# jjjkkyz/NU-NeRF

Hardware: AMD Instinct MI355X
Metric: train rays/sec (higher is better)
Workload: dtype f32

## Files before the change

nu_nerf_amd/csrc/gemm_tn.hip:

```cpp
#include "gemm_epi.h"

__device__ unsigned long long nu_dbg_clk[2];

#define NU_TN_BATCH_MAX 16
struct NuGemmTNBatch {
    NuGemmTN p[NU_TN_BATCH_MAX];
    int blk0[NU_TN_BATCH_MAX + 1];
    int n, pad_;
};
static __device__ __forceinline__ int tn_batch_decode(const NuGemmTNBatch& b, int tile_edge, int& bx, int& split) {
    int pi = 0;
    for (int i = 1; i < b.n; ++i) pi = ((int)blockIdx.x >= b.blk0[i]) ? i : pi;
    const int tiles = ((b.p[pi].N1 + tile_edge - 1) / tile_edge) * ((b.p[pi].N2 + tile_edge - 1) / tile_edge);
    const int local = (int)blockIdx.x - b.blk0[pi];
    split = local / tiles;
    bx = local - split * tiles;
    return pi;
}

template <bool BIG, int PREC>
static __device__ __forceinline__ void tn_body(const NuGemmTN& g, const int bx, const int split, const int grp) {
    constexpr bool BF16 = PREC == 1;
    constexpr bool SPLIT = PREC == 2;
    constexpr int kPlane = 128 * NT_LDSH;
    __shared__ __attribute__((aligned(16))) float smem[SPLIT ? 1 : 2][SPLIT ? 3 * kPlane : 128 * NT_LDS];
    __bf16* const hA = reinterpret_cast<__bf16*>(&smem[0][0]);
    __bf16* const hB = hA + (SPLIT ? 3 : 1) * kPlane;

    const int tid = threadIdx.x;
    const int lane = tid & 63;
    const int wid = tid >> 6;
    const int wr = wid >> 1, wc = wid & 1;
    const int t2 = (g.N2 + 127) / 128;
    const int n1t = bx / t2, n2t = bx - n1t * t2;
    const int n1_0 = n1t * 128, n2_0 = n2t * 128;
    const int N1p = ((g.N1 + 127) / 128) * 128, N2p = t2 * 128;

    int rows_per = (g.P + g.S - 1) / g.S;
    rows_per = ((rows_per + TBK - 1) / TBK) * TBK;
    const int p_begin = split * rows_per;
    int p_end = p_begin + rows_per;
    p_end = p_end < g.P ? p_end : g.P;
    const int ntile = p_end > p_begin ? (p_end - p_begin + TBK - 1) / TBK : 0;
    const int npair = g.A1 ? 2 : 1;
    const int total = ntile * npair;

    const int c = tid & 127;
    const int kg = tid >> 7;
    const bool do_bias = (g.bias_slab != nullptr) && (n2t == 0);

    f32x16 acc[2][2];
#pragma unroll
    for (int i = 0; i < 2; ++i)
#pragma unroll
        for (int j = 0; j < 2; ++j)
#pragma unroll
            for (int r = 0; r < 16; ++r) acc[i][j][r] = 0.0f;

    f32x4 ra4[4], rb4[4];
    int nvalid = 16;
    bool pend_pair0 = true;
    float bs = 0.f;
    auto load_tile = [&](int t) {
        const int pair = t >= ntile ? 1 : 0;
        const int kt = t - pair * ntile;
        const bool a16 = BF16 && (g.bf16 & (pair ? NU_TN_A1_16 : NU_TN_A0_16)) != 0;
        const bool b16 = BF16 && (g.bf16 & (pair ? NU_TN_B1_16 : NU_TN_B0_16)) != 0;
        const unsigned eA = a16 ? 2u : 4u, eB = b16 ? 2u : 4u;
        const char* __restrict__ A = (const char*)(pair ? g.A1 : g.A0) + (long long)grp * (pair ? g.sA1 : g.sA0) * eA;
        const char* __restrict__ B = (const char*)(pair ? g.B1 : g.B0) + (long long)grp * (pair ? g.sB1 : g.sB0) * eB;
        const int lda = pair ? g.lda1 : g.lda0;
        const int ldb = pair ? g.ldb1 : g.ldb0;
        int ca = n1_0 + c, cb = n2_0 + c;
        ca = ca < lda ? ca : lda - 1;
        cb = cb < ldb ? cb : ldb - 1;
        const int pbase = p_begin + kt * TBK + kg * 16;
        nvalid = p_end - pbase;
        pend_pair0 = pair == 0;
#pragma unroll
        for (int i = 0; i < 4; ++i)
#pragma unroll
            for (int e = 0; e < 4; ++e) {
                int pr = pbase + 4 * i + e;
                pr = pr < p_end ? pr : p_end - 1;
                const char* pa;
                const char* pb;
                if (BIG) {
                    pa = A + ((long long)pr * lda + ca) * eA;
                    pb = B + ((long long)pr * ldb + cb) * eB;
                } else {
                    pa = A + ((unsigned)pr * (unsigned)lda + (unsigned)ca) * eA;
                    pb = B + ((unsigned)pr * (unsigned)ldb + (unsigned)cb) * eB;
                }
                ra4[i][e] = a16 ? __uint_as_float((unsigned)*reinterpret_cast<const unsigned short*>(pa) << 16) : *reinterpret_cast<const float*>(pa);
                rb4[i][e] = b16 ? __uint_as_float((unsigned)*reinterpret_cast<const unsigned short*>(pb) << 16) : *reinterpret_cast<const float*>(pb);
            }
    };
    auto store_tile = [&]() {
#pragma unroll
        for (int i = 0; i < 4; ++i)
#pragma unroll
// ... 655 lines not shown
        TN_SLOT(F1, 2, TN_LD2(1, 2))
        TN_SLOT(F1, 3, TN_READS(F0, cur, 2))
        TN_SLOT(F0, 0, TN_ST(2))
        TN_SLOT(F0, 1, TN_ST(3))
        TN_SLOT(F0, 2, TN_LD2(2, 0))
        TN_SLOT(F0, 3, TN_READS(F1, cur, 3))
        __syncthreads();
        TN_SLOT(F1, 0, TN_LD2(2, 2))
        TN_SLOT(F1, 1, TN_LD2(3, 0))
        TN_SLOT(F1, 2, TN_LD2(3, 2))
        TN_SLOT(F1, 3, TN_READS(F0, cur ^ 1, 0))
        nvalid = nvalid_ld; pend_pair0 = pair0_ld;
        cur ^= 1;
    }
#undef TN_PIN
#undef TN_M
#undef TN_SLOT
#undef TN_SLOT_
#undef TN_RDA
#undef TN_RDB
#undef TN_READS
#undef TN_LD2
#undef TN_ST

    float* __restrict__ slab = g.slab + (long long)grp * g.sSlab + (long long)split * N1p * N2p;
#pragma unroll
    for (int tm = 0; tm < 2; ++tm)
#pragma unroll
        for (int tn = 0; tn < 4; ++tn) {
            const int col = n2_0 + wc * 128 + tn * 32 + li;
#pragma unroll
            for (int r = 0; r < 16; ++r) {
                const int row = n1_0 + wr * 64 + tm * 32 + (r & 3) + 8 * (r >> 2) + 4 * lh;
                slab[(long long)row * N2p + col] = acc[tm][tn][r];
            }
        }
    if (do_bias) {
        float* red = &smem[0][0][0];
        red[kg * T + c] = bs;
        __syncthreads();
        if (tid < T) g.bias_slab[(long long)grp * g.sBiasSlab + (long long)split * N1p + n1_0 + tid] = red[tid] + red[T + tid];
    }
}

template <bool BIG>
__global__ __launch_bounds__(512, 2) void gemm_tn2_kernel(NuGemmTN g) { tn2_body<BIG>(g, blockIdx.x, blockIdx.y, blockIdx.z); }
template <bool BIG>
__global__ __launch_bounds__(512, 2) void gemm_tn2b_kernel(NuGemmTNBatch b) {
    int bx, split;
    const int pi = tn_batch_decode(b, 256, bx, split);
    tn2_body<BIG>(b.p[pi], bx, split, 0);
}

static bool nu_tn_big_tile(int N1, int N2, int groups, int prec, int S) {
    if ((prec & 3) == 2 || (N1 % 256) != 0 || (N2 % 256) != 0) return false;
    return (long long)(N1 / 256) * (N2 / 256) * (groups > 0 ? groups : 1) * S >= 192;
}
extern "C" int nu_wgrad_pick_split(int P, int N1, int N2, int groups, int prec) {
    if (groups < 1) groups = 1;
    const int rows_min = P <= 8192 ? 128 : 256;
    const int cap = (P + rows_min - 1) / rows_min > 0 ? (P + rows_min - 1) / rows_min : 1;
    if ((N1 % 256) == 0 && (N2 % 256) == 0) {
        int S = 256 / ((N1 / 256) * (N2 / 256) * groups);
        if (S < 1) S = 1;
        if (S > cap) S = cap;
        if (nu_tn_big_tile(N1, N2, groups, prec, S)) return S;
    }
    int S = 512 / (nu_cdiv(N1, 128) * nu_cdiv(N2, 128) * groups);
    if (S < 1) S = 1;
    if (S > cap) S = cap;
    return S;
}

int nu_gemm_tn_launch(const NuGemmTN& g, hipStream_t stream) {
    if (g.N1 <= 0 || g.N2 <= 0 || g.S <= 0) return NU_ERR_ARG;
    if ((g.lda0 & 3) || (g.ldb0 & 3) || (g.A1 && ((g.lda1 & 3) || (g.ldb1 & 3)))) return NU_ERR_ARG;
    const int prec = g.bf16 & 3;
    if (prec == 3 || ((g.bf16 & ~3) && prec != 1)) return NU_ERR_ARG;
    const bool big_tile = nu_tn_big_tile(g.N1, g.N2, g.groups, g.bf16, g.S);
    const long long max_ld = (g.lda0 > g.ldb0 ? g.lda0 : g.ldb0) > (g.A1 ? (g.lda1 > g.ldb1 ? g.lda1 : g.ldb1) : 0)
                                 ? (g.lda0 > g.ldb0 ? g.lda0 : g.ldb0) : (g.lda1 > g.ldb1 ? g.lda1 : g.ldb1);
    const bool big = (long long)g.P * max_ld * 4 >= (1LL << 32);
    if (prec == 0 && big_tile) {
        dim3 grid2((g.N1 / 256) * (g.N2 / 256), g.S, g.groups > 0 ? g.groups : 1);
        if (big) hipLaunchKernelGGL((gemm_tn2_kernel<true>), grid2, dim3(512), 0, stream, g);
        else hipLaunchKernelGGL((gemm_tn2_kernel<false>), grid2, dim3(512), 0, stream, g);
        return nu_launch_status();
    }
    dim3 grid(nu_cdiv(g.N1, 128) * nu_cdiv(g.N2, 128), g.S, g.groups > 0 ? g.groups : 1), block(256);
    if (prec == 1) {
        auto ok = [](const float* p, int ld, bool h) { return p == nullptr || ((((uintptr_t)p) & 15) == 0 && ld >= 8 && (!h || (ld & 7) == 0)); };
        const bool vec = ok(g.A0, g.lda0, g.bf16 & NU_TN_A0_16) && ok(g.B0, g.ldb0, g.bf16 & NU_TN_B0_16) &&
                         ok(g.A1, g.lda1, g.bf16 & NU_TN_A1_16) && ok(g.B1, g.ldb1, g.bf16 & NU_TN_B1_16) &&
                         ((g.sA0 | g.sB0 | g.sA1 | g.sB1) & 7) == 0;
        if (vec) {
            if (big_tile) {
                dim3 grid2((g.N1 / 256) * (g.N2 / 256), g.S, g.groups > 0 ? g.groups : 1);
                hipLaunchKernelGGL(gemm_tn16x256_kernel, grid2, dim3(512), 0, stream, g);
            } else {
                hipLaunchKernelGGL(gemm_tn16_kernel, grid, block, 0, stream, g);
            }
            return nu_launch_status();
        }
    }
    if (big) {
        if (prec == 2) hipLaunchKernelGGL((gemm_tn_kernel<true, 2>), grid, block, 0, stream, g);
        else if (prec == 1) hipLaunchKernelGGL((gemm_tn_kernel<true, 1>), grid, block, 0, stream, g);
        else hipLaunchKernelGGL((gemm_tn_kernel<true, 0>), grid, block, 0, stream, g);
    } else {
        if (prec == 2) hipLaunchKernelGGL((gemm_tn_kernel<false, 2>), grid, block, 0, stream, g);
        else if (prec == 1) hipLaunchKernelGGL((gemm_tn_kernel<false, 1>), grid, block, 0, stream, g);
        else hipLaunchKernelGGL((gemm_tn_kernel<false, 0>), grid, block, 0, stream, g);
    }
    return nu_launch_status();
}

struct NuReduceBatch {
    NuReduceDesc d[NU_REDUCE_MAX];
    int n;
};

__global__ __launch_bounds__(256) void slab_reduce_batched_kernel(NuReduceBatch b) {
    __shared__ float red[256];
    int di = 0;
    for (int i = 1; i < b.n; ++i) di = ((int)blockIdx.x >= b.d[i].blk_begin) ? i : di;
    const float* __restrict__ slab = b.d[di].slab;
    float* __restrict__ out = b.d[di].out;
    const int S = b.d[di].S, N1 = b.d[di].N1, N2 = b.d[di].N2, rs = b.d[di].rs, G = b.d[di].G;
    const long long ss = b.d[di].ss;
    const int opb = 256 / G;
    const int o = threadIdx.x % opb, g = threadIdx.x / opb;
    const int idx = ((int)blockIdx.x - b.d[di].blk_begin) * opb + o;
    const bool live = idx < N1 * N2;
    float v = 0.f;
    int n1 = 0, n2 = 0;
    if (live) {
        n1 = idx / N2;
        n2 = idx - n1 * N2;
        const float* p = slab + (long long)n1 * rs + n2;
        float s0 = 0.f, s1 = 0.f, s2 = 0.f, s3 = 0.f;
        int s = g;
        for (; s + 3 * G < S; s += 4 * G) {
            s0 += p[(long long)s * ss];
            s1 += p[(long long)(s + G) * ss];
            s2 += p[(long long)(s + 2 * G) * ss];
            s3 += p[(long long)(s + 3 * G) * ss];
        }
        for (; s < S; s += G) s0 += p[(long long)s * ss];
        v = (s0 + s1) + (s2 + s3);
    }
    if (G > 1) {
        red[threadIdx.x] = v;
        __syncthreads();
        if (g == 0)
            for (int gg = 1; gg < G; ++gg) v += red[gg * opb + o];
    }
    if (live && g == 0) {
        float* q = out + (long long)n1 * b.d[di].ldo + n2;
        v *= b.d[di].alpha;
        *q = b.d[di].accumulate ? *q + v : v;
    }
}

static int nu_reduce_launch_chunk(const NuReduceDesc* descs, int n, hipStream_t stream) {
    NuReduceBatch b;
    int blocks = 0;
    for (int i = 0; i < n; ++i) {
        b.d[i] = descs[i];
        const long long nout = (long long)descs[i].N1 * descs[i].N2;
        int G = 1;
        while (G < 16 && nout * G < 16384 && 2 * G <= descs[i].S) G *= 2;
// ... 83 lines not shown
                            dW + z * sW, ldw, 1.0f, 0);
        if (rc == NU_OK && db)
            rc = nu_reduce_push(descs, ndesc, cap, g.bias_slab + z * bias_per, g.S, g.N1, 1, 1, N1p, db + z * sDb, 1, 1.0f, 0);
    }
    return rc;
}

extern "C" int nu_wgrad(const NuGemmTN* gin, float* dW, int ldw, long long sW, float* db, long long sDb,
                        void* workspace, long long workspace_bytes, hipStream_t stream) {
    const int groups = gin->groups > 0 ? gin->groups : 1;
    if (groups > NU_REDUCE_MAX / 2) return NU_ERR_ARG;
    NuReduceDesc descs[NU_REDUCE_MAX];
    int n = 0;
    int rc = nu_wgrad_enqueue(gin, dW, ldw, sW, db, sDb, workspace, workspace_bytes, descs, &n, NU_REDUCE_MAX, stream);
    if (rc) return rc;
    return nu_slab_reduce_batched(descs, n, stream);
}

extern "C" int nu_wgrad_item_size(void) { return (int)sizeof(NuWgradItem); }

static int ctx_reduce_now(NuOpCtx* c, hipStream_t stream) {
    if (c->ndesc > 0) {
        const int rc = nu_slab_reduce_batched(c->descs, c->ndesc, stream);
        if (rc != NU_OK) return rc;
        c->ndesc = 0;
    }
    c->arena_off = 0;
    return NU_OK;
}
extern "C" int nu_wgrad_flush(NuOpCtx* c, hipStream_t stream);
extern "C" int nu_ctx_reduce(NuOpCtx* c, hipStream_t stream) { return ctx_reduce_now(c, stream); }
extern "C" int nu_ctx_flush(NuOpCtx* c, hipStream_t stream) {
    const int rc = nu_wgrad_flush(c, stream);
    if (rc != NU_OK) return rc;
    return ctx_reduce_now(c, stream);
}
int nu_ctx_take(NuOpCtx* c, long long nbytes, int ndesc_needed, hipStream_t stream, float** out, long long* out_bytes) {
    const long long n = (nbytes + 255) / 256 * 64;
    if (n > c->arena_floats) return NU_ERR_WORKSPACE;
    if (c->arena_off + n > c->arena_floats || c->ndesc + ndesc_needed > c->cap) {
        if (c->forked) return NU_ERR_WORKSPACE;
        const int rc = ctx_reduce_now(c, stream);
        if (rc != NU_OK) return rc;
    }
    *out = c->arena + c->arena_off;
    *out_bytes = n * 4;
    c->arena_off += n;
    return NU_OK;
}
void nu_ctx_ev_begin(NuOpCtx* c, hipStream_t stream) {
    if (c->ev && c->nev + 2 <= c->ev_cap) (void)hipEventRecord(static_cast<hipEvent_t>(c->ev[c->nev]), stream);
}
void nu_ctx_ev_end(NuOpCtx* c, hipStream_t stream, double kind, double flops, double bytes) {
    if (c->ev && c->nev + 2 <= c->ev_cap) {
        (void)hipEventRecord(static_cast<hipEvent_t>(c->ev[c->nev + 1]), stream);
        double* m = c->ev_meta + 3 * (c->nev / 2);
        m[0] = kind; m[1] = flops; m[2] = bytes;
        c->nev += 2;
    }
}

static inline bool tn_item_big(const NuGemmTN& g) {
    const long long m0 = g.lda0 > g.ldb0 ? g.lda0 : g.ldb0, m1 = g.A1 ? (g.lda1 > g.ldb1 ? g.lda1 : g.ldb1) : 0;
    return (long long)g.P * (m0 > m1 ? m0 : m1) * 4 >= (1LL << 32);
}

static int wgrad_launch_batch(NuOpCtx* c, NuWgradItem* it, const int* idx, int m, int klass, hipStream_t stream) {
    long long bytes = 0;
    int ndesc = 0, nprob = 0;
    for (int k = 0; k < m; ++k) {
        const NuGemmTN& g = it[idx[k]].g;
        bytes += (nu_wgrad_workspace_bytes(g.N1, g.N2, g.S, g.groups) + 255) / 256 * 256;
        ndesc += g.groups * (it[idx[k]].db ? 2 : 1);
        nprob += g.groups;
    }
    if (nprob > NU_TN_BATCH_MAX) return NU_ERR_ARG;
    float* ws;
    long long nb;
    int rc = nu_ctx_take(c, bytes, ndesc, stream, &ws, &nb);
    if (rc != NU_OK) return rc;
    NuGemmTNBatch b;
    int np = 0, blocks = 0;
    double flops = 0, abytes = 0;
    const int edge = klass == 2 ? 256 : 128;
    for (int k = 0; k < m; ++k) {
        NuWgradItem& w = it[idx[k]];
        const NuGemmTN& g = w.g;
        const int N1p = nu_rup(g.N1, 128), N2p = nu_rup(g.N2, 128);
        const long long slab_per = (long long)g.S * N1p * N2p, bias_per = (long long)g.S * N1p;
        float* slab = ws;
        float* bias_slab = w.db ? slab + slab_per * g.groups : nullptr;
        ws += (nu_wgrad_workspace_bytes(g.N1, g.N2, g.S, g.groups) + 255) / 256 * 64;
        for (int z = 0; z < g.groups; ++z) {
            NuGemmTN& q = b.p[np];
            q = g;
            q.groups = 1;
            q.A0 = g.A0 + z * g.sA0; q.B0 = g.B0 + z * g.sB0;
            q.A1 = g.A1 ? g.A1 + z * g.sA1 : nullptr; q.B1 = g.B1 ? g.B1 + z * g.sB1 : nullptr;
            q.slab = slab + z * slab_per; q.bias_slab = bias_slab ? bias_slab + z * bias_per : nullptr;
            q.sSlab = 0; q.sBiasSlab = 0;
            b.blk0[np++] = blocks;
            blocks += nu_cdiv(g.N1, edge) * nu_cdiv(g.N2, edge) * g.S;
            rc = nu_reduce_push(c->descs, &c->ndesc, c->cap, q.slab, g.S, g.N1, g.N2, N2p, (long long)N1p * N2p, w.dW + z * w.sW, w.ldw, 1.0f, 0);
            if (rc == NU_OK && w.db)
                rc = nu_reduce_push(c->descs, &c->ndesc, c->cap, q.bias_slab, g.S, g.N1, 1, 1, N1p, w.db + z * w.sDb, 1, 1.0f, 0);
            if (rc != NU_OK) return rc;
        }
        flops += w.flops; abytes += w.bytes;
    }
    b.blk0[np] = blocks;
    b.n = np; b.pad_ = 0;
    nu_ctx_ev_begin(c, stream);
    if (klass == 2) hipLaunchKernelGGL((gemm_tn2b_kernel<false>), dim3(blocks), dim3(512), 0, stream, b);
    else hipLaunchKernelGGL((gemm_tnb_kernel<false>), dim3(blocks), dim3(256), 0, stream, b);
    rc = nu_launch_status();
    nu_ctx_ev_end(c, stream, 1.0, flops, abytes);
    return rc;
}

static int wgrad_launch_single(NuOpCtx* c, NuWgradItem& w, hipStream_t stream) {
    NuGemmTN& g = w.g;
    g.S = nu_wgrad_pick_split(g.P, g.N1, g.N2, g.groups, g.bf16 & 3);
    float* ws;
    long long nb;
    int rc = nu_ctx_take(c, nu_wgrad_workspace_bytes(g.N1, g.N2, g.S, g.groups), 2 * g.groups, stream, &ws, &nb);
    if (rc != NU_OK) return rc;
    nu_ctx_ev_begin(c, stream);
    rc = nu_wgrad_enqueue(&g, w.dW, w.ldw, w.sW, w.db, w.sDb, ws, nb, c->descs, &c->ndesc, c->cap, stream);
    nu_ctx_ev_end(c, stream, 1.0, w.flops, w.bytes);
    return rc;
}

extern "C" int nu_wgrad_flush(NuOpCtx* c, hipStream_t stream) {
    const int n = c->npend;
    if (n <= 0 || c->pend == nullptr) return NU_OK;
    NuWgradItem* it = c->pend;
    c->npend = 0;
    int klass[NU_WGRAD_QUEUE_MAX];
    if (n > NU_WGRAD_QUEUE_MAX) return NU_ERR_ARG;
    int pmax = 0;
    for (int i = 0; i < n; ++i) {
        NuGemmTN& g = it[i].g;
        if (g.groups < 1) g.groups = 1;
        klass[i] = ((g.bf16 & 3) == 0 && (g.bf16 & ~3) == 0 && !tn_item_big(g) && g.groups <= NU_TN_BATCH_MAX) ? 1 : 0;
        if (klass[i] && g.P > pmax) pmax = g.P;
    }
    const int rows_min = pmax <= 8192 ? 128 : 256;
    auto plan = [&](int k, int edge, int target) -> long long {
        long long work = 0;
        for (int i = 0; i < n; ++i)
            if (klass[i] == k) work += (long long)it[i].g.P * nu_cdiv(it[i].g.N1, edge) * nu_cdiv(it[i].g.N2, edge) * it[i].g.groups;
        if (work == 0) return 0;
        long long rows = nu_cdivl(work, target);
        rows = rows < rows_min ? rows_min : rows;
        rows = nu_cdivl(rows, TBK) * TBK;
        while (true) {
            long long wgs = 0;
            for (int i = 0; i < n; ++i)
                if (klass[i] == k) wgs += nu_cdivl(it[i].g.P, rows) * nu_cdiv(it[i].g.N1, edge) * nu_cdiv(it[i].g.N2, edge) * it[i].g.groups;
            if (wgs <= target || rows >= (1LL << 30)) { for (int i = 0; i < n; ++i) if (klass[i] == k) it[i].g.S = (int)nu_cdivl(it[i].g.P, rows); return wgs; }
            rows += TBK;
        }
    };
    for (int i = 0; i < n; ++i)
        if (klass[i] == 1 && (it[i].g.N1 % 256) == 0 && (it[i].g.N2 % 256) == 0) klass[i] = 2;
    if (plan(2, 256, 256) < 192)
        for (int i = 0; i < n; ++i) if (klass[i] == 2) klass[i] = 1;
    plan(1, 128, 1024);
    for (int i = 0; i < n; ++i)
        if (klass[i] == 0) { const int rc = wgrad_launch_single(c, it[i], stream); if (rc != NU_OK) return rc; }
    for (int k = 2; k >= 1; --k) {
        int idx[NU_WGRAD_QUEUE_MAX], m = 0, nprob = 0;
        long long bytes = 0;
        for (int i = 0; i <= n; ++i) {
            const bool mine = i < n && klass[i] == k;
            long long need = 0;
            if (mine) need = (nu_wgrad_workspace_bytes(it[i].g.N1, it[i].g.N2, it[i].g.S, it[i].g.groups) + 255) / 256 * 256;
            const bool full = mine && m > 0 && (nprob + it[i].g.groups > NU_TN_BATCH_MAX || bytes + need > c->arena_floats * 4);
            if ((i == n || full) && m > 0) {
                const int rc = wgrad_launch_batch(c, it, idx, m, k, stream);
                if (rc != NU_OK) return rc;
                m = 0; nprob = 0; bytes = 0;
            }
            if (mine) { idx[m++] = i; nprob += it[i].g.groups; bytes += need; }
        }
    }
    return NU_OK;
}

extern "C" int nu_wgrad_defer(NuOpCtx* c, const NuGemmTN* g, float* dW, int ldw, long long sW, float* db, long long sDb, double flops,
                              double bytes, hipStream_t stream) {
    if (g->P <= 0) return NU_OK;
    NuWgradItem w;
    w.g = *g; w.dW = dW; w.ldw = ldw; w.pad_ = 0; w.sW = sW; w.db = db; w.sDb = sDb; w.flops = flops; w.bytes = bytes;
    if (w.g.groups < 1) w.g.groups = 1;
    if (c->pend == nullptr || c->pend_cap <= 0) return wgrad_launch_single(c, w, stream);
    if (c->npend >= c->pend_cap || c->npend >= NU_WGRAD_QUEUE_MAX) {
        const int rc = nu_wgrad_flush(c, stream);
        if (rc != NU_OK) return rc;
    }
    c->pend[c->npend++] = w;
    return NU_OK;
}

__global__ __launch_bounds__(256) void mfma_peak_kernel(float* out, int iters) {
    f32x16 a0 = {}, a1 = {}, a2 = {}, a3 = {};
    const unsigned long long c0 = clock64(), w0 = wall_clock64();
    float x = (float)threadIdx.x * 1e-3f, y = 1.0f + (float)blockIdx.x * 1e-6f;
    for (int i = 0; i < iters; ++i) {
        a0 = __builtin_amdgcn_mfma_f32_32x32x2f32(x, y, a0, 0, 0, 0);
        a1 = __builtin_amdgcn_mfma_f32_32x32x2f32(y, x, a1, 0, 0, 0);
        a2 = __builtin_amdgcn_mfma_f32_32x32x2f32(x, x, a2, 0, 0, 0);
        a3 = __builtin_amdgcn_mfma_f32_32x32x2f32(y, y, a3, 0, 0, 0);
    }
    float s = 0.f;
    for (int r = 0; r < 16; ++r) s += a0[r] + a1[r] + a2[r] + a3[r];
    if (s == 123.456f) out[0] = s;
    if (blockIdx.x == 0 && threadIdx.x == 0) { nu_dbg_clk[0] = clock64() - c0; nu_dbg_clk[1] = wall_clock64() - w0; }
}
extern "C" double nu_debug_clock_mhz(void) {
    unsigned long long h[2] = {0, 0};
    if (hipMemcpyFromSymbol(h, HIP_SYMBOL(nu_dbg_clk), sizeof(h)) != hipSuccess || h[1] == 0) return -1.0;
    return (double)h[0] / (double)h[1] * 100.0;
}
extern "C" int nu_debug_mfma_peak(float* out, int blocks, int iters, hipStream_t stream) {
    hipLaunchKernelGGL(mfma_peak_kernel, dim3(blocks), dim3(256), 0, stream, out, iters);
    return nu_launch_status();
}
```

Before: 98870.

## Add hand-scheduled fp32 MFMA weight-gradient kernels with fused bias row-sum

Adds new 256- and 128-tile fp32 weight-gradient GEMM kernels that interleave global loads, LDS stores and MFMA issues by hand, using sched barriers and a double-buffered LDS. The bias gradient is computed from per-tile row sums inside the same loop. Both the single-launch and the batched paths route eligible fp32 problems (aligned, under 4 GB, no bf16) to these kernels through two new klass values. The goal is to hide memory latency behind MFMA work, at the cost of rigid hand scheduling, extra register pressure and a new, untested correctness surface.

```diff
diff --git a/nu_nerf_amd/csrc/gemm_tn.hip b/nu_nerf_amd/csrc/gemm_tn.hip
--- a/nu_nerf_amd/csrc/gemm_tn.hip
+++ b/nu_nerf_amd/csrc/gemm_tn.hip
@@ -1,22 +1,8 @@
 #include "gemm_epi.h"
+#include "wgrad_rm.h"
 
 __device__ unsigned long long nu_dbg_clk[2];
 
-#define NU_TN_BATCH_MAX 16
-struct NuGemmTNBatch {
-    NuGemmTN p[NU_TN_BATCH_MAX];
-    int blk0[NU_TN_BATCH_MAX + 1];
-    int n, pad_;
-};
-static __device__ __forceinline__ int tn_batch_decode(const NuGemmTNBatch& b, int tile_edge, int& bx, int& split) {
-    int pi = 0;
-    for (int i = 1; i < b.n; ++i) pi = ((int)blockIdx.x >= b.blk0[i]) ? i : pi;
-    const int tiles = ((b.p[pi].N1 + tile_edge - 1) / tile_edge) * ((b.p[pi].N2 + tile_edge - 1) / tile_edge);
-    const int local = (int)blockIdx.x - b.blk0[pi];
-    split = local / tiles;
-    bx = local - split * tiles;
-    return pi;
-}
 
 template <bool BIG, int PREC>
 static __device__ __forceinline__ void tn_body(const NuGemmTN& g, const int bx, const int split, const int grp) {
@@ -838,11 +824,13 @@
                                  ? (g.lda0 > g.ldb0 ? g.lda0 : g.ldb0) : (g.lda1 > g.ldb1 ? g.lda1 : g.ldb1);
     const bool big = (long long)g.P * max_ld * 4 >= (1LL << 32);
     if (prec == 0 && big_tile) {
+        if (!big && nu_wgrad_rm_ok(g) && (((uintptr_t)g.slab) & 15) == 0 && (g.sSlab & 3) == 0) return nu_wgrad_rm256_launch(g, stream);
         dim3 grid2((g.N1 / 256) * (g.N2 / 256), g.S, g.groups > 0 ? g.groups : 1);
         if (big) hipLaunchKernelGGL((gemm_tn2_kernel<true>), grid2, dim3(512), 0, stream, g);
         else hipLaunchKernelGGL((gemm_tn2_kernel<false>), grid2, dim3(512), 0, stream, g);
         return nu_launch_status();
     }
+    if (prec == 0 && !big && nu_wgrad_rm_ok(g) && (((uintptr_t)g.slab) & 15) == 0 && (g.sSlab & 3) == 0) return nu_wgrad_rm128_launch(g, stream);
     dim3 grid(nu_cdiv(g.N1, 128) * nu_cdiv(g.N2, 128), g.S, g.groups > 0 ? g.groups : 1), block(256);
     if (prec == 1) {
         auto ok = [](const float* p, int ld, bool h) { return p == nullptr || ((((uintptr_t)p) & 15) == 0 && ld >= 8 && (!h || (ld & 7) == 0)); };
@@ -1092,7 +1080,7 @@
     NuGemmTNBatch b;
     int np = 0, blocks = 0;
     double flops = 0, abytes = 0;
-    const int edge = klass == 2 ? 256 : 128;
+    const int edge = (klass == 2 || klass == 3) ? 256 : 128;
     for (int k = 0; k < m; ++k) {
         NuWgradItem& w = it[idx[k]];
         const NuGemmTN& g = w.g;
@@ -1121,9 +1109,13 @@
     b.blk0[np] = blocks;
     b.n = np; b.pad_ = 0;
     nu_ctx_ev_begin(c, stream);
-    if (klass == 2) hipLaunchKernelGGL((gemm_tn2b_kernel<false>), dim3(blocks), dim3(512), 0, stream, b);
-    else hipLaunchKernelGGL((gemm_tnb_kernel<false>), dim3(blocks), dim3(256), 0, stream, b);
-    rc = nu_launch_status();
+    if (klass >= 3) {
+        rc = klass == 3 ? nu_wgrad_rm256_launch_batch(b, blocks, stream) : nu_wgrad_rm128_launch_batch(b, blocks, stream);
+    } else {
+        if (klass == 2) hipLaunchKernelGGL((gemm_tn2b_kernel<false>), dim3(blocks), dim3(512), 0, stream, b);
+        else hipLaunchKernelGGL((gemm_tnb_kernel<false>), dim3(blocks), dim3(256), 0, stream, b);
+        rc = nu_launch_status();
+    }
     nu_ctx_ev_end(c, stream, 1.0, flops, abytes);
     return rc;
 }
@@ -1178,8 +1170,10 @@
         for (int i = 0; i < n; ++i) if (klass[i] == 2) klass[i] = 1;
     plan(1, 128, 1024);
     for (int i = 0; i < n; ++i)
+        if (klass[i] >= 1 && nu_wgrad_rm_ok(it[i].g)) klass[i] = klass[i] == 2 ? 3 : 4;
+    for (int i = 0; i < n; ++i)
         if (klass[i] == 0) { const int rc = wgrad_launch_single(c, it[i], stream); if (rc != NU_OK) return rc; }
-    for (int k = 2; k >= 1; --k) {
+    for (int k = 4; k >= 1; --k) {
         int idx[NU_WGRAD_QUEUE_MAX], m = 0, nprob = 0;
         long long bytes = 0;
         for (int i = 0; i <= n; ++i) {
diff --git a/nu_nerf_amd/csrc/wgrad_rm.h b/nu_nerf_amd/csrc/wgrad_rm.h
--- /dev/null
+++ b/nu_nerf_amd/csrc/wgrad_rm.h
@@ -0,0 +1,26 @@
+#pragma once
+#include "gemm.h"
+
+#define NU_TN_BATCH_MAX 16
+struct NuGemmTNBatch {
+    NuGemmTN p[NU_TN_BATCH_MAX];
+    int blk0[NU_TN_BATCH_MAX + 1];
+    int n, pad_;
+};
+#ifdef __HIPCC__
+static __device__ __forceinline__ int tn_batch_decode(const NuGemmTNBatch& b, int tile_edge, int& bx, int& split) {
+    int pi = 0;
+    for (int i = 1; i < b.n; ++i) pi = ((int)blockIdx.x >= b.blk0[i]) ? i : pi;
+    const int tiles = ((b.p[pi].N1 + tile_edge - 1) / tile_edge) * ((b.p[pi].N2 + tile_edge - 1) / tile_edge);
+    const int local = (int)blockIdx.x - b.blk0[pi];
+    split = local / tiles;
+    bx = local - split * tiles;
+    return pi;
+}
+#endif
+
+bool nu_wgrad_rm_ok(const NuGemmTN& g);
+int nu_wgrad_rm256_launch(const NuGemmTN& g, hipStream_t stream);
+int nu_wgrad_rm256_launch_batch(const NuGemmTNBatch& b, int blocks, hipStream_t stream);
+int nu_wgrad_rm128_launch(const NuGemmTN& g, hipStream_t stream);
+int nu_wgrad_rm128_launch_batch(const NuGemmTNBatch& b, int blocks, hipStream_t stream);
diff --git a/nu_nerf_amd/csrc/wgrad_rm.hip b/nu_nerf_amd/csrc/wgrad_rm.hip
--- /dev/null
+++ b/nu_nerf_amd/csrc/wgrad_rm.hip
@@ -0,0 +1,431 @@
+#include <type_traits>
+
+#include "gemm_epi.h"
+#include "wgrad_rm.h"
+
+typedef float f32x2 __attribute__((ext_vector_type(2)));
+
+static __device__ __forceinline__ float rm_add(float a, float b) {
+    float r;
+    asm volatile("v_add_f32 %0, %1, %2" : "=v"(r) : "v"(a), "v"(b));
+    return r;
+}
+
+static __device__ __forceinline__ void rm256_body(const NuGemmTN& g, const int bx, const int split, const int grp) {
+    constexpr int T = 256;
+    __shared__ __attribute__((aligned(16))) float smem[2][2][TBK * T];
+    __shared__ __attribute__((aligned(16))) float rsb[2][8][T];
+    const int tid = threadIdx.x;
+    const int lane = tid & 63;
+    const int wid = __builtin_amdgcn_readfirstlane(tid >> 6);
+    const int wr = wid >> 1, wc = wid & 1;
+    const int t2 = g.N2 / T;
+    const int n1t = bx / t2, n2t = bx - n1t * t2;
+    const int n1_0 = n1t * T, n2_0 = n2t * T;
+    const int N1p = g.N1, N2p = g.N2;
+
+    int rows_per = (g.P + g.S - 1) / g.S;
+    rows_per = ((rows_per + TBK - 1) / TBK) * TBK;
+    const int p_begin = split * rows_per;
+    int p_end = p_begin + rows_per;
+    p_end = p_end < g.P ? p_end : g.P;
+    const int ntile = p_end > p_begin ? (p_end - p_begin + TBK - 1) / TBK : 0;
+    const int npair = g.A1 ? 2 : 1;
+    const int total = ntile * npair;
+
+    const int c = tid & (T - 1);
+    const int kg = tid / T;
+    const bool do_bias = (g.bias_slab != nullptr) && (n2t == 0);
+
+    f32x16 acc[2][4];
+#pragma unroll
+    for (int i = 0; i < 2; ++i)
+#pragma unroll
+        for (int j = 0; j < 4; ++j)
+#pragma unroll
+            for (int r = 0; r < 16; ++r) acc[i][j][r] = 0.0f;
+    float bs = 0.f;
+
+    if (total > 0) {
+        f32x4 ra[4], rb[4];
+        int pend_pr0 = 0;
+        bool pend_pair0 = true;
+        const char* __restrict__ ldA = nullptr;
+        const char* __restrict__ ldB = nullptr;
+        unsigned ld_lda4 = 0, ld_ldb4 = 0, ld_qa = 0, ld_qb = 0;
+        int ld_pr0 = 0;
+        bool ld_pair0 = true;
+        auto ld_begin = [&](int t) {
+            const int pair = t >= ntile ? 1 : 0;
+            const int kt = t - pair * ntile;
+            ldA = (const char*)(pair ? g.A1 + (long long)grp * g.sA1 : g.A0 + (long long)grp * g.sA0);
+            ldB = (const char*)(pair ? g.B1 + (long long)grp * g.sB1 : g.B0 + (long long)grp * g.sB0);
+            const int lda = pair ? g.lda1 : g.lda0, ldb = pair ? g.ldb1 : g.ldb0;
+            int qa = n1_0 / 4 + lane, qb = n2_0 / 4 + lane;
+            const int qam = (g.N1 - 1) / 4 < lda / 4 - 1 ? (g.N1 - 1) / 4 : lda / 4 - 1;
+            const int qbm = (g.N2 - 1) / 4 < ldb / 4 - 1 ? (g.N2 - 1) / 4 : ldb / 4 - 1;
+            qa = qa < qam ? qa : qam;
+            qb = qb < qbm ? qb : qbm;
+            ld_qa = (unsigned)qa * 16u; ld_qb = (unsigned)qb * 16u;
+            ld_lda4 = (unsigned)lda * 4u; ld_ldb4 = (unsigned)ldb * 4u;
+            ld_pr0 = p_begin + kt * TBK + 4 * wid;
+            ld_pair0 = pair == 0;
+        };
+        auto ld_row = [&](bool isA, int e) {
+            int pr = ld_pr0 + e;
+            pr = pr < p_end ? pr : p_end - 1;
+            if (isA) ra[e] = *reinterpret_cast<const f32x4*>(ldA + (size_t)((unsigned)pr * ld_lda4) + ld_qa);
+            else rb[e] = *reinterpret_cast<const f32x4*>(ldB + (size_t)((unsigned)pr * ld_ldb4) + ld_qb);
+        };
+        auto ld_done = [&]() { pend_pr0 = ld_pr0; pend_pair0 = ld_pair0; };
+        auto st_zero = [&](bool isA) {
+#pragma unroll
+            for (int e = 0; e < 4; ++e) {
+                const bool ok = pend_pr0 + e < p_end;
+#pragma unroll
+                for (int q = 0; q < 4; ++q) {
+                    if (isA) ra[e][q] = ok ? ra[e][q] : 0.f;
+                    else rb[e][q] = ok ? rb[e][q] : 0.f;
+                }
+            }
+        };
+        auto st_rs = [&](int par) {
+            f32x4 rs;
+#pragma unroll
+            for (int q = 0; q < 4; ++q) rs[q] = rm_add(rm_add(ra[0][q], ra[1][q]), rm_add(ra[2][q], ra[3][q]));
+            *reinterpret_cast<f32x4*>(&rsb[par][wid][4 * lane]) = rs;
+        };
+        auto st_write = [&](bool isA, int st, int e) {
+            if (isA) *reinterpret_cast<f32x4*>(&smem[st][0][(4 * wid + e) * T + 4 * lane]) = ra[e];
+            else *reinterpret_cast<f32x4*>(&smem[st][1][(4 * wid + e) * T + 4 * lane]) = rb[e];
+        };
+        auto bias_add = [&](int par, bool on) {
+#pragma unroll
+            for (int i = 0; i < 4; ++i) {
+                const float v = rsb[par][4 * kg + i][c];
+                bs += on ? v : 0.f;
+            }
+        };
+
+        ld_begin(0);
+#pragma unroll
+        for (int e = 0; e < 4; ++e) { ld_row(true, e); ld_row(false, e); }
+        ld_done();
+        st_zero(true); st_zero(false);
+        st_rs(0);
+#pragma unroll
+        for (int e = 0; e < 4; ++e) { st_write(true, 0, e); st_write(false, 0, e); }
+        ld_begin(total > 1 ? 1 : 0);
+#pragma unroll
+        for (int e = 0; e < 4; ++e) { ld_row(true, e); ld_row(false, e); }
+        ld_done();
+        __syncthreads();
+        bias_add(0, do_bias);
+
+        const int li = lane & 31, lh = lane >> 5;
+        const int a_off = 4 * lh * T + wr * 64 + 2 * li;
+        const int b_off = 4 * lh * T + wc * 128 + 4 * li;
+        struct FragT { f32x2 a; f32x4 b; };
+        FragT F0, F1;
+        F0.a = *reinterpret_cast<const f32x2*>(&smem[0][0][a_off]);
+        F0.b = *reinterpret_cast<const f32x4*>(&smem[0][1][b_off]);
+        int cur = 0;
+        bool bias_on = false;
+#define RM_PIN __builtin_amdgcn_sched_barrier(0);
+#define RM_M(F, i, j) acc[i][j] = __builtin_amdgcn_mfma_f32_32x32x2f32(F.a[i], F.b[j], acc[i][j], 0, 0, 0); RM_PIN
+#define RM_SLOT(F, ...) RM_SLOT_(F, __VA_ARGS__)
+#define RM_SLOT_(F, X0, X1, X2, X3, X4, X5, X6)                                                   \
+    RM_M(F, 0, 0) X0; RM_PIN RM_M(F, 0, 1) X1; RM_PIN RM_M(F, 0, 2) X2; RM_PIN RM_M(F, 0, 3) X3; RM_PIN     \
+    RM_M(F, 1, 0) X4; RM_PIN RM_M(F, 1, 1) X5; RM_PIN RM_M(F, 1, 2) X6; RM_PIN RM_M(F, 1, 3)
+#define RM_RDA(F, ST, s) F.a = *reinterpret_cast<const f32x2*>(&smem[ST][0][a_off + (((s) >> 2) * 8 + ((s) & 3)) * T])
+#define RM_RDB(F, ST, s) F.b = *reinterpret_cast<const f32x4*>(&smem[ST][1][b_off + (((s) >> 2) * 8 + ((s) & 3)) * T])
+#define RM_RD(F, ST, s) RM_RDA(F, ST, s), RM_RDB(F, ST, s)
+        for (int t = 0; t < total; ++t) {
+            bias_on = do_bias && pend_pair0 && t + 1 < total;
+            RM_SLOT(F0, RM_RD(F1, cur, 1), st_zero(true), st_rs(cur ^ 1), ld_begin(t + 2 < total ? t + 2 : total - 1), st_write(true, cur ^ 1, 0), st_write(true, cur ^ 1, 1))
+            RM_SLOT(F1, RM_RD(F0, cur, 2), st_write(true, cur ^ 1, 2), st_write(true, cur ^ 1, 3), ld_row(true, 0), ld_row(true, 1), st_zero(false))
+            RM_SLOT(F0, RM_RD(F1, cur, 3), ld_row(true, 2), ld_row(true, 3), st_write(false, cur ^ 1, 0), st_write(false, cur ^ 1, 1), st_write(false, cur ^ 1, 2))
+            RM_SLOT(F1, RM_RD(F0, cur, 4), st_write(false, cur ^ 1, 3), ld_row(false, 0), ld_row(false, 1), ld_row(false, 2), ld_row(false, 3))
+            RM_SLOT(F0, RM_RD(F1, cur, 5), (void)0, (void)0, (void)0, (void)0, (void)0)
+            RM_SLOT(F1, RM_RD(F0, cur, 6), (void)0, (void)0, (void)0, (void)0, (void)0)
+            RM_SLOT(F0, RM_RD(F1, cur, 7), (void)0, (void)0, (void)0, (void)0, (void)0)
+            RM_SLOT(F1, RM_RD(F0, cur, 8), (void)0, (void)0, (void)0, (void)0, (void)0)
+            RM_SLOT(F0, RM_RD(F1, cur, 9), (void)0, (void)0, (void)0, (void)0, (void)0)
+            RM_SLOT(F1, RM_RD(F0, cur, 10), (void)0, (void)0, (void)0, (void)0, (void)0)
+            RM_SLOT(F0, RM_RD(F1, cur, 11), (void)0, (void)0, (void)0, (void)0, (void)0)
+            RM_SLOT(F1, RM_RD(F0, cur, 12), (void)0, (void)0, (void)0, (void)0, (void)0)
+            RM_SLOT(F0, RM_RD(F1, cur, 13), (void)0, (void)0, (void)0, (void)0, (void)0)
+            RM_SLOT(F1, RM_RD(F0, cur, 14), (void)0, (void)0, (void)0, (void)0, (void)0)
+            RM_SLOT(F0, RM_RD(F1, cur, 15), (void)0, (void)0, (void)0, (void)0, (void)0)
+            __syncthreads();
+            RM_SLOT(F1, RM_RD(F0, cur ^ 1, 0), bias_add(cur ^ 1, bias_on), (void)0, (void)0, (void)0, (void)0)
+            ld_done();
+            cur ^= 1;
+        }
+#undef RM_PIN
+#undef RM_M
+#undef RM_SLOT
+#undef RM_SLOT_
+#undef RM_RDA
+#undef RM_RDB
+#undef RM_RD
+    }
+
+    const int li = lane & 31, lh = lane >> 5;
+    float* __restrict__ slab = g.slab + (long long)grp * g.sSlab + (long long)split * N1p * N2p;
+    const int col = n2_0 + wc * 128 + 4 * li;
+#pragma unroll
+    for (int i = 0; i < 2; ++i)
+#pragma unroll
+        for (int r = 0; r < 16; ++r) {
+            const int row = n1_0 + wr * 64 + 2 * ((r & 3) + 8 * (r >> 2) + 4 * lh) + i;
+            f32x4 v;
+            v[0] = acc[i][0][r]; v[1] = acc[i][1][r]; v[2] = acc[i][2][r]; v[3] = acc[i][3][r];
+            *reinterpret_cast<f32x4*>(&slab[(long long)row * N2p + col]) = v;
+        }
+    if (do_bias) {
+        __syncthreads();
+        float* red = &smem[0][0][0];
+        red[kg * T + c] = bs;
+        __syncthreads();
+        if (tid < T) g.bias_slab[(long long)grp * g.sBiasSlab + (long long)split * N1p + n1_0 + tid] = red[tid] + red[T + tid];
+    }
+}
+
+__global__ __launch_bounds__(512, 2) void wgrad_rm256_kernel(NuGemmTN g) { rm256_body(g, blockIdx.x, blockIdx.y, blockIdx.z); }
+__global__ __launch_bounds__(512, 2) void wgrad_rm256b_kernel(NuGemmTNBatch b) {
+    int bx, split;
+    const int pi = tn_batch_decode(b, 256, bx, split);
+    rm256_body(b.p[pi], bx, split, 0);
+}
+
+static __device__ __forceinline__ void rm128_body(const NuGemmTN& g, const int bx, const int split, const int grp) {
+    constexpr int T = 128;
+    __shared__ __attribute__((aligned(16))) float smem[2][2][TBK * T];
+    __shared__ __attribute__((aligned(16))) float rsb[2][8][T];
+    const int tid = threadIdx.x;
+    const int lane = tid & 63;
+    const int wid = __builtin_amdgcn_readfirstlane(tid >> 6);
+    const int wr = wid >> 1, wc = wid & 1;
+    const int t2 = (g.N2 + T - 1) / T;
+    const int n1t = bx / t2, n2t = bx - n1t * t2;
+    const int n1_0 = n1t * T, n2_0 = n2t * T;
+    const int N1p = ((g.N1 + 127) / 128) * 128, N2p = t2 * 128;
+
+    int rows_per = (g.P + g.S - 1) / g.S;
+    rows_per = ((rows_per + TBK - 1) / TBK) * TBK;
+    const int p_begin = split * rows_per;
+    int p_end = p_begin + rows_per;
+    p_end = p_end < g.P ? p_end : g.P;
+    const int ntile = p_end > p_begin ? (p_end - p_begin + TBK - 1) / TBK : 0;
+    const int npair = g.A1 ? 2 : 1;
+    const int total = ntile * npair;
+
+    const int c = tid & (T - 1);
+    const int kg = tid / T;
+    const bool do_bias = (g.bias_slab != nullptr) && (n2t == 0);
+    const bool live = (n1_0 + wr * 64 < g.N1) && (n2_0 + wc * 64 < g.N2);
+
+    f32x16 acc[2][2];
+#pragma unroll
+    for (int i = 0; i < 2; ++i)
+#pragma unroll
+        for (int j = 0; j < 2; ++j)
+#pragma unroll
+            for (int r = 0; r < 16; ++r) acc[i][j][r] = 0.0f;
+    float bs = 0.f;
+    const int li = lane & 31, lh = lane >> 5;
+
+    if (total > 0) {
+        f32x4 ra[4], rb[4];
+        int pend_pr = 0;
+        bool pend_pair0 = true;
+        const char* __restrict__ ldA = nullptr;
+        const char* __restrict__ ldB = nullptr;
+        unsigned ld_lda4 = 0, ld_ldb4 = 0, ld_qa = 0, ld_qb = 0;
+        int ld_pr = 0;
+        bool ld_pair0 = true;
+        auto ld_begin = [&](int t) {
+            const int pair = t >= ntile ? 1 : 0;
+            const int kt = t - pair * ntile;
+            ldA = (const char*)(pair ? g.A1 + (long long)grp * g.sA1 : g.A0 + (long long)grp * g.sA0);
+            ldB = (const char*)(pair ? g.B1 + (long long)grp * g.sB1 : g.B0 + (long long)grp * g.sB0);
+            const int lda = pair ? g.lda1 : g.lda0, ldb = pair ? g.ldb1 : g.ldb0;
+            int qa = n1_0 / 4 + li, qb = n2_0 / 4 + li;
+            const int qam = (g.N1 - 1) / 4 < lda / 4 - 1 ? (g.N1 - 1) / 4 : lda / 4 - 1;
+            const int qbm = (g.N2 - 1) / 4 < ldb / 4 - 1 ? (g.N2 - 1) / 4 : ldb / 4 - 1;
+            qa = qa < qam ? qa : qam;
+            qb = qb < qbm ? qb : qbm;
+            ld_qa = (unsigned)qa * 16u; ld_qb = (unsigned)qb * 16u;
+            ld_lda4 = (unsigned)lda * 4u; ld_ldb4 = (unsigned)ldb * 4u;
+            ld_pr = p_begin + kt * TBK + 8 * wid + 4 * lh;
+            ld_pair0 = pair == 0;
+        };
+        auto ld_row = [&](bool isA, int e) {
+            int pr = ld_pr + e;
+            pr = pr < p_end ? pr : p_end - 1;
+            if (isA) ra[e] = *reinterpret_cast<const f32x4*>(ldA + (size_t)((unsigned)pr * ld_lda4 + ld_qa));
+            else rb[e] = *reinterpret_cast<const f32x4*>(ldB + (size_t)((unsigned)pr * ld_ldb4 + ld_qb));
+        };
+        auto ld_done = [&]() { pend_pr = ld_pr; pend_pair0 = ld_pair0; };
+        auto st_zero = [&](bool isA) {
+#pragma unroll
+            for (int e = 0; e < 4; ++e) {
+                const bool ok = pend_pr + e < p_end;
+#pragma unroll
+                for (int q = 0; q < 4; ++q) {
+                    if (isA) ra[e][q] = ok ? ra[e][q] : 0.f;
+                    else rb[e][q] = ok ? rb[e][q] : 0.f;
+                }
+            }
+        };
+        auto st_rs = [&](int par) {
+            f32x4 rs;
+#pragma unroll
+            for (int q = 0; q < 4; ++q) rs[q] = rm_add(rm_add(ra[0][q], ra[1][q]), rm_add(ra[2][q], ra[3][q]));
+            *reinterpret_cast<f32x4*>(&rsb[par][2 * wid + lh][4 * li]) = rs;
+        };
+        auto st_write = [&](bool isA, int st, int e) {
+            if (isA) *reinterpret_cast<f32x4*>(&smem[st][0][(8 * wid + 4 * lh + e) * T + 4 * li]) = ra[e];
+            else *reinterpret_cast<f32x4*>(&smem[st][1][(8 * wid + 4 * lh + e) * T + 4 * li]) = rb[e];
+        };
+        auto bias_add = [&](int par, bool on) {
+#pragma unroll
+            for (int i = 0; i < 4; ++i) {
+                const float v = rsb[par][4 * kg + i][c];
+                bs += on ? v : 0.f;
+            }
+        };
+
+        ld_begin(0);
+#pragma unroll
+        for (int e = 0; e < 4; ++e) { ld_row(true, e); ld_row(false, e); }
+        ld_done();
+        st_zero(true); st_zero(false);
+        st_rs(0);
+#pragma unroll
+        for (int e = 0; e < 4; ++e) { st_write(true, 0, e); st_write(false, 0, e); }
+        ld_begin(total > 1 ? 1 : 0);
+#pragma unroll
+        for (int e = 0; e < 4; ++e) { ld_row(true, e); ld_row(false, e); }
+        ld_done();
+        __syncthreads();
+        bias_add(0, do_bias);
+
+        const int a_off = 4 * lh * T + wr * 64 + 2 * li;
+        const int b_off = 4 * lh * T + wc * 64 + 2 * li;
+        struct FragT { f32x2 a; f32x2 b; };
+        FragT F0, F1;
+        F0.a = *reinterpret_cast<const f32x2*>(&smem[0][0][a_off]);
+        F0.b = *reinterpret_cast<const f32x2*>(&smem[0][1][b_off]);
+        F1 = F0;
+        int cur = 0;
+        bool bias_on = false;
+#define RM_PIN __builtin_amdgcn_sched_barrier(0);
+#define RM_M(F, i, j) if constexpr (LIVE) acc[i][j] = __builtin_amdgcn_mfma_f32_32x32x2f32(F.a[i], F.b[j], acc[i][j], 0, 0, 0); RM_PIN
+#define RM_SLOT(F, ...) RM_SLOT_(F, __VA_ARGS__)
+#define RM_SLOT_(F, R0, R1, X2, X3) RM_M(F, 0, 0) if constexpr (LIVE) { R0; } RM_PIN RM_M(F, 0, 1) if constexpr (LIVE) { R1; } RM_PIN RM_M(F, 1, 0) X2; RM_PIN RM_M(F, 1, 1) X3; RM_PIN
+#define RM_RDA(F, ST, s) F.a = *reinterpret_cast<const f32x2*>(&smem[ST][0][a_off + (((s) >> 2) * 8 + ((s) & 3)) * T])
+#define RM_RDB(F, ST, s) F.b = *reinterpret_cast<const f32x2*>(&smem[ST][1][b_off + (((s) >> 2) * 8 + ((s) & 3)) * T])
+#define RM_RD(F, ST, s) RM_RDA(F, ST, s), RM_RDB(F, ST, s)
+        auto chunks = [&](auto live_c) {
+            constexpr bool LIVE = decltype(live_c)::value;
+            for (int t = 0; t < total; ++t) {
+                bias_on = do_bias && pend_pair0 && t + 1 < total;
+                RM_SLOT(F0, RM_RD(F1, cur, 1), st_zero(true), st_rs(cur ^ 1))
+                RM_SLOT(F1, RM_RD(F0, cur, 2), ld_begin(t + 2 < total ? t + 2 : total - 1), st_write(true, cur ^ 1, 0))
+                RM_SLOT(F0, RM_RD(F1, cur, 3), st_write(true, cur ^ 1, 1), st_write(true, cur ^ 1, 2))
+                RM_SLOT(F1, RM_RD(F0, cur, 4), st_write(true, cur ^ 1, 3), ld_row(true, 0))
+                RM_SLOT(F0, RM_RD(F1, cur, 5), ld_row(true, 1), ld_row(true, 2))
+                RM_SLOT(F1, RM_RD(F0, cur, 6), ld_row(true, 3), st_zero(false))
+                RM_SLOT(F0, RM_RD(F1, cur, 7), st_write(false, cur ^ 1, 0), st_write(false, cur ^ 1, 1))
+                RM_SLOT(F1, RM_RD(F0, cur, 8), st_write(false, cur ^ 1, 2), st_write(false, cur ^ 1, 3))
+                RM_SLOT(F0, RM_RD(F1, cur, 9), ld_row(false, 0), ld_row(false, 1))
+                RM_SLOT(F1, RM_RD(F0, cur, 10), ld_row(false, 2), ld_row(false, 3))
+                RM_SLOT(F0, RM_RD(F1, cur, 11), (void)0, (void)0)
+                RM_SLOT(F1, RM_RD(F0, cur, 12), (void)0, (void)0)
+                RM_SLOT(F0, RM_RD(F1, cur, 13), (void)0, (void)0)
+                RM_SLOT(F1, RM_RD(F0, cur, 14), (void)0, (void)0)
+                RM_SLOT(F0, RM_RD(F1, cur, 15), (void)0, (void)0)
+                __syncthreads();
+                RM_SLOT(F1, RM_RD(F0, cur ^ 1, 0), bias_add(cur ^ 1, bias_on), (void)0)
+                ld_done();
+                cur ^= 1;
+            }
+        };
+        if (live) chunks(std::true_type{});
+        else chunks(std::false_type{});
+#undef RM_PIN
+#undef RM_M
+#undef RM_SLOT
+#undef RM_SLOT_
+#undef RM_RDA
+#undef RM_RDB
+#undef RM_RD
+    }
+
+    if (live) {
+        float* __restrict__ slab = g.slab + (long long)grp * g.sSlab + (long long)split * N1p * N2p;
+        const int col = n2_0 + wc * 64 + 2 * li;
+#pragma unroll
+        for (int i = 0; i < 2; ++i)
+#pragma unroll
+            for (int r = 0; r < 16; ++r) {
+                const int row = n1_0 + wr * 64 + 2 * ((r & 3) + 8 * (r >> 2) + 4 * lh) + i;
+                f32x2 v;
+                v[0] = acc[i][0][r]; v[1] = acc[i][1][r];
+                *reinterpret_cast<f32x2*>(&slab[(long long)row * N2p + col]) = v;
+            }
+    }
+    if (do_bias) {
+        __syncthreads();
+        float* red = &smem[0][0][0];
+        red[kg * T + c] = bs;
+        __syncthreads();
+        if (tid < T) g.bias_slab[(long long)grp * g.sBiasSlab + (long long)split * N1p + n1_0 + tid] = red[tid] + red[T + tid];
+    }
+}
+
+__global__ __launch_bounds__(256, 2) void wgrad_rm128_kernel(NuGemmTN g) { rm128_body(g, blockIdx.x, blockIdx.y, blockIdx.z); }
+__global__ __launch_bounds__(256, 2) void wgrad_rm128b_kernel(NuGemmTNBatch b) {
+    int bx, split;
+    const int pi = tn_batch_decode(b, 128, bx, split);
+    rm128_body(b.p[pi], bx, split, 0);
+}
+
+bool nu_wgrad_rm_ok(const NuGemmTN& g) {
+    if ((g.bf16 & 3) != 0 || (g.bf16 & ~3) != 0) return false;
+    const int groups = g.groups > 0 ? g.groups : 1;
+    auto ok = [&](const float* p, int ld, long long s, int n) {
+        if (p == nullptr) return true;
+        if ((((uintptr_t)p) & 15) != 0 || (ld & 3) != 0 || ld < n) return false;
+        if (groups > 1 && (s & 3) != 0) return false;
+        return (long long)g.P * ld * 4 < (1LL << 32);
+    };
+    if (g.A1 != nullptr && g.B1 == nullptr) return false;
+    return ok(g.A0, g.lda0, g.sA0, g.N1) && ok(g.B0, g.ldb0, g.sB0, g.N2) && ok(g.A1, g.lda1, g.sA1, g.N1) && ok(g.B1, g.ldb1, g.sB1, g.N2);
+}
+
+int nu_wgrad_rm256_launch(const NuGemmTN& g, hipStream_t stream) {
+    if ((g.N1 % 256) != 0 || (g.N2 % 256) != 0 || !nu_wgrad_rm_ok(g)) return NU_ERR_ARG;
+    dim3 grid((g.N1 / 256) * (g.N2 / 256), g.S, g.groups > 0 ? g.groups : 1);
+    hipLaunchKernelGGL(wgrad_rm256_kernel, grid, dim3(512), 0, stream, g);
+    return nu_launch_status();
+}
+
+int nu_wgrad_rm256_launch_batch(const NuGemmTNBatch& b, int blocks, hipStream_t stream) {
+    hipLaunchKernelGGL(wgrad_rm256b_kernel, dim3(blocks), dim3(512), 0, stream, b);
+    return nu_launch_status();
+}
+
+int nu_wgrad_rm128_launch(const NuGemmTN& g, hipStream_t stream) {
+    if (!nu_wgrad_rm_ok(g)) return NU_ERR_ARG;
+    dim3 grid(nu_cdiv(g.N1, 128) * nu_cdiv(g.N2, 128), g.S, g.groups > 0 ? g.groups : 1);
+    hipLaunchKernelGGL(wgrad_rm128_kernel, grid, dim3(256), 0, stream, g);
+    return nu_launch_status();
+}
+
+int nu_wgrad_rm128_launch_batch(const NuGemmTNBatch& b, int blocks, hipStream_t stream) {
+    hipLaunchKernelGGL(wgrad_rm128b_kernel, dim3(blocks), dim3(256), 0, stream, b);
+    return nu_launch_status();
+}
```

New measurement: 100,400, median of 6. +1.5%, better.
